# Autobot37/weatherforecastingtoolkit

Measured on AMD Instinct MI355X. Metric: SEVIR 384x384 frames/sec (AE train step), higher is better.
Workload: dtype f32; 1 GPU; experiments/ae_v2 conv AE (ae_64x8x8_lin.PosAwareAE_TF, img_size=384), 1x384x384 synthetic SEVIR frames, batch 32/GPU, fp32, fwd + L1 + bwd + AdamW + cosine-warmup LR; batch_per_gpu=32, global_batch=32, img_size=384, parallelism=dp1, params=215033281

## Files before the change

### include/wfae.h

```cpp
#ifndef WFAE_H
#define WFAE_H

#include <stddef.h>
#include <stdint.h>

#ifdef __cplusplus
extern "C" {
#endif

typedef void* wfae_stream_t;

typedef enum {
  WFAE_OK = 0,
  WFAE_ERR_BAD_SHAPE = -1,
  WFAE_ERR_NULL_POINTER = -2,
  WFAE_ERR_WORKSPACE = -3,
  WFAE_ERR_LAUNCH = -4,
  WFAE_ERR_UNSUPPORTED = -5
} wfae_status;

int wfae_version(void);
const char* wfae_last_error_string(void);
size_t wfae_workspace_bytes(int64_t max_weight_elems);

// ... 4 lines not shown
int wfae_set_split_gemm(int on);
int wfae_get_split_gemm(void);

int wfae_set_c1n(int on);
int wfae_get_c1n(void);

int wfae_conv1x1_fwd(const float* x, const float* w, const float* bias, const float* res,
                     int64_t res_img_stride, float* y, int NB, int Cin, int Cout, int HW,
                     wfae_stream_t stream);
int wfae_conv1x1_fwd_stats(const float* x, const float* w, const float* bias, const float* res,
                           int64_t res_img_stride, float* y, int NB, int Cin, int Cout, int HW,
                           double* stat_part, int64_t stat_capacity, int* stat_rows, wfae_stream_t stream);
int wfae_conv1x1_fwd_bnact(const float* x, const float* bn_scale, const float* bn_shift, const float* w,
                           const float* bias, const float* res, int64_t res_img_stride, float* y, int NB, int Cin,
                           int Cout, int HW, double* stat_part, int64_t stat_capacity, int* stat_rows,
                           wfae_stream_t stream);
int wfae_conv1x1_bwd_weight_bnact(const float* dy, const float* x, const float* bn_scale, const float* bn_shift,
                                  float* dw, int NB, int Cin, int Cout, int HW, int accumulate, void* ws,
                                  size_t ws_bytes, wfae_stream_t stream);
int wfae_conv1x1_bwd_data(const float* dy, const float* w, float* dx, int NB, int Cin, int Cout,
                          int HW, wfae_stream_t stream);
int wfae_conv1x1_bwd_weight(const float* dy, const float* x, float* dw, int NB, int Cin, int Cout,
                            int HW, int accumulate, void* ws, size_t ws_bytes, wfae_stream_t stream);

int wfae_c1r_supported(int M, int K, int HW);
int wfae_c1r_stat_rows(int M, int K, int NB, int HW);
int wfae_c1r_fwd(const float* w, int64_t w_sm, int64_t w_sk, const float* x, const float* pro_scale, const float* pro_shift,
                 const float* res, float* y, int NB, int K, int M, int HW, double* stat_part, int64_t stat_capacity,
                 int* stat_rows, wfae_stream_t stream);
int wfae_c1r_bnred_supported(int M, int K, int HW);
int wfae_c1r_bnred(const float* w, int64_t w_sm, int64_t w_sk, const float* dt, const float* x, const float* bn_scale,
                   const float* bn_shift, const float* save_mean, const float* save_invstd, float* da, int NB, int K, int M, int HW,
                   double* part, int64_t part_capacity, int* part_rows, wfae_stream_t stream);
int wfae_bn_act_bwd_from_rows(const double* part, int rows, int C, float* dgamma, float* dbeta, int accumulate, void* ws,
                              size_t ws_bytes, wfae_stream_t stream);
int wfae_c1r_bndx(const float* w, int64_t w_sm, int64_t w_sk, const float* dt, const float* x, const float* gamma,
                  const float* bn_scale, const float* bn_shift, const float* save_mean, const float* save_invstd, const float* coef,
                  const float* res, float* dx, int NB, int K, int M, int HW, int training, wfae_stream_t stream);
int wfae_c1rb_supported(int M, int K, int HW);
int wfae_c1rb_stat_rows(int M, int K, int NB, int HW);
int wfae_c1rb_fwd(const float* w, int64_t w_sm, int64_t w_sk, const uint16_t* x, const float* pro_scale, const float* pro_shift,
                  const uint16_t* res, uint16_t* y, int NB, int K, int M, int HW, double* stat_part, int64_t stat_capacity,
                  int* stat_rows, wfae_stream_t stream);
int wfae_c1w_supported(int Cin, int Cout, int HW);
int wfae_c1w_bwd_weight(const float* dy, const float* x, const float* bn_scale, const float* bn_shift, float* dw, int NB, int Cin,
                        int Cout, int HW, int accumulate, void* ws, size_t ws_bytes, wfae_stream_t stream);
int wfae_c1w_bwd_weight_bf16(const uint16_t* dy, const uint16_t* x, const float* bn_scale, const float* bn_shift, float* dw, int NB,
                             int Cin, int Cout, int HW, int accumulate, void* ws, size_t ws_bytes, wfae_stream_t stream);
int wfae_set_c1wd(int on);
int wfae_get_c1wd(void);
int wfae_c1wd_supported(int C, int mid, int HW);
int wfae_c1wd_bwd(const float* dy, const float* t2, const float* bn_scale, const float* bn_shift, const float* w3, float* dw3,
                  float* da3, int NB, int C, int mid, int HW, int accumulate, void* ws, size_t ws_bytes, wfae_stream_t stream);
int wfae_set_c1ws(int on);
int wfae_get_c1ws(void);
int wfae_c1ws_supported(int C, int mid, int HW);
int wfae_c1ws_stat_rows(int C, int mid, int NB, int HW, size_t ws_bytes);
int wfae_c1ws_bwd(const float* x, const float* dt1, const float* bn_scale, const float* bn_shift, const float* save_mean,
                  const float* save_invstd, const float* w1, float* dw1, double* part, int64_t part_capacity, int* part_rows, int NB,
                  int C, int mid, int HW, int accumulate, void* ws, size_t ws_bytes, wfae_stream_t stream);
int wfae_linear_fwd(const float* x, const float* w, const float* bias, float* y, int B, int In,
                    int Out, void* ws, size_t ws_bytes, wfae_stream_t stream);
int wfae_linear_bwd_data(const float* dy, const float* w, float* dx, int B, int In, int Out,
                         wfae_stream_t stream);
int wfae_linear_bwd_weight(const float* dy, const float* x, float* dw, int B, int In, int Out,
                           int accumulate, wfae_stream_t stream);
int wfae_linear_bwd_data_splitk(const float* dy, const float* w, float* dx, int B, int In, int Out, void* ws,
                                size_t ws_bytes, wfae_stream_t stream);
int wfae_linear_bwd_weight_splitk(const float* dy, const float* x, float* dw, int B, int In, int Out, int accumulate,
                                  void* ws, size_t ws_bytes, wfae_stream_t stream);

int wfae_conv4x4s2_down(const float* hi, const float* w, float* lo, int NB, int Chi, int Clo,
                        int Hlo, int Wlo, wfae_stream_t stream);
int wfae_conv4x4s2_up(const float* lo, const float* w, float* hi, int NB, int Chi, int Clo, int Hlo,
                      int Wlo, void* ws, size_t ws_bytes, wfae_stream_t stream);
int wfae_conv4x4s2_wgrad(const float* lo, const float* hi, float* dw, int NB, int Chi, int Clo,
                         int Hlo, int Wlo, int accumulate, void* ws, size_t ws_bytes,
                         wfae_stream_t stream);

int wfae_dconv_fwd(const float* x, const float* w, const float* bias, float* y, int NB, int Cin,
                   int Cout, int H, int W, int KS, int stride, int pad, int groups,
                   wfae_stream_t stream);
int wfae_dconv_bwd_data(const float* dy, const float* w, float* dx, int NB, int Cin, int Cout,
                        int H, int W, int KS, int pad, int groups, wfae_stream_t stream);
int wfae_dconv_bwd_weight(const float* dy, const float* x, float* dw, int NB, int Cin, int Cout,
                          int H, int W, int KS, int stride, int pad, int groups, int accumulate,
                          void* ws, size_t ws_bytes, wfae_stream_t stream);

int wfae_gconv3x3_fwd(const float* x, const float* w, float* y, int NB, int C, int H, int W, int groups,
                      int transposed, void* ws, size_t ws_bytes, wfae_stream_t stream);
int wfae_gconv3x3_bwd_weight(const float* dy, const float* x, float* dw, int NB, int C, int H, int W,
                             int groups, int accumulate, void* ws, size_t ws_bytes, wfae_stream_t stream);

int wfae_bn_stats_train(const float* x, int NB, int C, int HW, const float* gamma,
                        const float* beta, float eps, float momentum, float* running_mean,
                        float* running_var, float* save_mean, float* save_invstd, float* scale,
                        float* shift, void* ws, size_t ws_bytes, wfae_stream_t stream);
int wfae_bn_stats_from_rows(const double* stat_part, int rows, int NB, int C, int HW, const float* gamma,
                            const float* beta, float eps, float momentum, float* running_mean,
                            float* running_var, float* save_mean, float* save_invstd, float* scale,
                            float* shift, void* ws, size_t ws_bytes, wfae_stream_t stream);
int wfae_bn_fold_eval(const float* gamma, const float* beta, const float* running_mean,
                      const float* running_var, float eps, float* save_mean, float* save_invstd,
                      float* scale, float* shift, int C, wfae_stream_t stream);
int wfae_bn_act_fwd(const float* x, const float* scale, const float* shift, float* y, int NB, int C,
                    int HW, int act, wfae_stream_t stream);
// ... 361 lines not shown
```

### weatherforecastingtoolkit_amd/csrc/c1wd.hip

```cpp
#include "common.h"
#include <atomic>
#include <stdlib.h>
#include <type_traits>

using namespace wfae;

namespace {

typedef float f32x4 __attribute__((ext_vector_type(4)));
typedef float f32x16 __attribute__((ext_vector_type(16)));
typedef __bf16 bf16x8 __attribute__((ext_vector_type(8)));
typedef short s16x4 __attribute__((ext_vector_type(4)));
typedef short s16x8 __attribute__((ext_vector_type(8)));
typedef unsigned u32x4 __attribute__((ext_vector_type(4)));
typedef unsigned u32x2 __attribute__((ext_vector_type(2)));

struct C1WDP {
  const float* dy;
  const float* t2;
  const float* w3;
  const float* pro_scale;
  const float* pro_shift;
  float* slab;
  float* da;
  int HW;
  int cpi;
  int kc;
};

constexpr int DNT = 512, DBK = 32;

__device__ __forceinline__ unsigned off_row(int r, int c) { return (unsigned)(r * 64 + ((c ^ ((r >> 2) & 3)) << 4)); }

__device__ __forceinline__ void split_pair(float a, float b, unsigned& h, unsigned& m, unsigned& l) {
  h = pack_bf16(a, b);
  const float ra = a - bf16_lo(h), rb = b - bf16_hi(h);
  m = pack_bf16(ra, rb);
  l = pack_bf16(ra - bf16_lo(m), rb - bf16_hi(m));
}

template <int C>
__global__ __launch_bounds__(DNT, C == 128 ? 4 : 2) void c1wd_kernel(C1WDP p) {
  constexpr int M = C / 4;
  constexpr int TM = C / 128;
  constexpr int WQ = M / 32;
  constexpr int NDW = 4 * WQ;
  constexpr bool BOTH = NDW == 8;
  constexpr int KCH = C / 32;
  constexpr int LPR = 8;
  constexpr int P_LD = C * LPR, Q_LD = M * LPR;
  constexpr int P_IT = P_LD / DNT;
  static_assert(P_LD % DNT == 0 && Q_LD <= DNT, "loader");
  constexpr int A_PLANE_B = C * 64, B_PLANE_B = M * 64;
  constexpr int A_STAGE_B = 3 * A_PLANE_B, STAGE_B = 3 * (A_PLANE_B + B_PLANE_B);
  __shared__ __attribute__((aligned(16))) unsigned char smem[2 * STAGE_B];
  const int t = threadIdx.x, lane = t & 63;
  const int wave = __builtin_amdgcn_readfirstlane(t >> 6);
  const int img = blockIdx.x / p.cpi, chunk = blockIdx.x - img * p.cpi;
  const int k_begin = chunk * p.kc;
  const int k_end = min(p.HW, k_begin + p.kc);
  const int nsteps = (k_end - k_begin) / DBK;
  const bool do_dw = BOTH || wave < NDW, do_da = BOTH || wave >= NDW;

  const float* Pb = p.dy + (long)img * C * p.HW + k_begin;
  const float* Qb = p.t2 + (long)img * M * p.HW + k_begin;
  const float* p_src[P_IT];
  unsigned p_dst[P_IT];
#pragma unroll
  for (int j = 0; j < P_IT; ++j) {
    const int idx = t + j * DNT, r = idx / LPR, e = idx % LPR;
    p_src[j] = Pb + (long)r * p.HW + e * 4;
    p_dst[j] = off_row(r, e >> 1) + (unsigned)((e & 1) * 8);
  }
  const bool q_on = Q_LD == DNT || t < Q_LD;
  const int q_r = q_on ? t / LPR : 0, q_e = t % LPR;
  const float* q_src = Qb + (long)q_r * p.HW + q_e * 4;
  const unsigned q_dst = off_row(q_r, q_e >> 1) + (unsigned)((q_e & 1) * 8);
  const float q_s = p.pro_scale[q_r], q_h = p.pro_shift[q_r];
  u32x4 rp[P_IT], rq;
  auto load_global = [&]() {
#pragma unroll
    for (int j = 0; j < P_IT; ++j) rp[j] = *reinterpret_cast<const u32x4*>(p_src[j]);
    if (q_on) rq = *reinterpret_cast<const u32x4*>(q_src);
  };
  auto advance = [&](bool more) {
#pragma unroll
    for (int j = 0; j < P_IT; ++j) p_src[j] += more ? DBK : 0;
    q_src += more ? DBK : 0;
  };
  auto put = [&](unsigned char* base, int plane_b, unsigned dst, u32x4 r, bool act, float s, float h) {
    const unsigned u0 = r[0], u1 = r[1], u2 = r[2], u3 = r[3];
    float v0 = __uint_as_float(u0), v1 = __uint_as_float(u1), v2 = __uint_as_float(u2), v3 = __uint_as_float(u3);
    if (act) {
      v0 = gelu_f(fmaf(v0, s, h)); v1 = gelu_f(fmaf(v1, s, h));
      v2 = gelu_f(fmaf(v2, s, h)); v3 = gelu_f(fmaf(v3, s, h));
    }
    unsigned h0, m0, l0, h1, m1, l1;
    split_pair(v0, v1, h0, m0, l0);
    split_pair(v2, v3, h1, m1, l1);
    *reinterpret_cast<u32x2*>(base + dst) = u32x2{h0, h1};
    *reinterpret_cast<u32x2*>(base + plane_b + dst) = u32x2{m0, m1};
    *reinterpret_cast<u32x2*>(base + 2 * plane_b + dst) = u32x2{l0, l1};
  };
  auto store_lds = [&](int buf) {
    unsigned char* s = smem + buf * STAGE_B;
#pragma unroll
    for (int j = 0; j < P_IT; ++j) put(s, A_PLANE_B, p_dst[j], rp[j], false, 0.f, 0.f);
    if (q_on) put(s + A_STAGE_B, B_PLANE_B, q_dst, rq, true, q_s, q_h);
  };

  const int wm0 = (BOTH ? (wave >> 1) : (wave & 3)) * (32 * TM), wn0 = BOTH ? (wave & 1) * 32 : 0;
  const int r31 = lane & 31, lh = lane >> 5;
  const unsigned a_rd = (unsigned)((wm0 + r31) * 64), b_rd = (unsigned)((wn0 + r31) * 64);
  const int a_x = (r31 >> 2) & 3;
  f32x16 acc[TM];
  struct Frag {
    bf16x8 a[TM][3], b[3];
  };
  auto read_frag = [&](Frag& f, int buf, int ks) {
    const unsigned char* s = smem + buf * STAGE_B;
    const unsigned a_c = (unsigned)(((2 * ks + lh) ^ a_x) << 4);
#pragma unroll
    for (int i = 0; i < TM; ++i)
#pragma unroll
      for (int pl = 0; pl < 3; ++pl)
        f.a[i][pl] = *reinterpret_cast<const bf16x8*>(s + pl * A_PLANE_B + a_rd + i * (32 * 64) + a_c);
#pragma unroll
    for (int pl = 0; pl < 3; ++pl) f.b[pl] = *reinterpret_cast<const bf16x8*>(s + A_STAGE_B + pl * B_PLANE_B + b_rd + a_c);
  };
  auto mfma_frag = [&](const Frag& f) {
#pragma unroll
    for (int i = 0; i < TM; ++i) {
      f32x16 c = acc[i];
      c = __builtin_amdgcn_mfma_f32_32x32x16_bf16(f.a[i][2], f.b[0], c, 0, 0, 0);
      c = __builtin_amdgcn_mfma_f32_32x32x16_bf16(f.a[i][0], f.b[2], c, 0, 0, 0);
      c = __builtin_amdgcn_mfma_f32_32x32x16_bf16(f.a[i][1], f.b[1], c, 0, 0, 0);
      c = __builtin_amdgcn_mfma_f32_32x32x16_bf16(f.a[i][1], f.b[0], c, 0, 0, 0);
      c = __builtin_amdgcn_mfma_f32_32x32x16_bf16(f.a[i][0], f.b[1], c, 0, 0, 0);
      c = __builtin_amdgcn_mfma_f32_32x32x16_bf16(f.a[i][0], f.b[0], c, 0, 0, 0);
      acc[i] = c;
    }
  };

  const int dtile = BOTH ? wave : (wave & 3);
  const int mt = dtile >> 1, pt = dtile & 1;
  const int n16 = lane & 15, kg = lane >> 4, tq = n16 >> 2, tp = n16 & 3;
  bf16x8 wa[KCH][3];
  auto load_weights = [&]() {
#pragma unroll
    for (int ch = 0; ch < KCH; ++ch) {
      const float* src = p.w3 + (long)(32 * ch + 8 * kg) * M + 16 * mt + n16;
      float v[8];
#pragma unroll
      for (int e = 0; e < 8; ++e) v[e] = src[e * M];
      u32x4 h, m, l;
#pragma unroll
      for (int e = 0; e < 4; ++e) {
        unsigned qh, qm, ql;
        split_pair(v[2 * e], v[2 * e + 1], qh, qm, ql);
        h[e] = qh; m[e] = qm; l[e] = ql;
      }
      wa[ch][0] = __builtin_bit_cast(bf16x8, h);
      wa[ch][1] = __builtin_bit_cast(bf16x8, m);
      wa[ch][2] = __builtin_bit_cast(bf16x8, l);
    }
  };
  unsigned tr_rd[2];
#pragma unroll
  for (int hf = 0; hf < 2; ++hf) tr_rd[hf] = off_row(8 * kg + 4 * hf + tq, 2 * pt + (tp >> 1)) + 8u * (unsigned)(tp & 1);
  float* const da_dst = p.da + ((long)img * M + 16 * mt + 4 * kg) * p.HW + k_begin + 16 * pt + n16;
  auto da_step = [&](int buf, int st) {
    const unsigned char* s = smem + buf * STAGE_B;
    constexpr int PA[6] = {2, 0, 1, 1, 0, 0}, PB[6] = {0, 2, 1, 0, 1, 0};
    f32x4 d = {0.f, 0.f, 0.f, 0.f};
#pragma unroll
    for (int ch = 0; ch < KCH; ++ch) {
      bf16x8 b[3];
#pragma unroll
      for (int pl = 0; pl < 3; ++pl) {
        s16x4 part[2];
#pragma unroll
        for (int hf = 0; hf < 2; ++hf)
          part[hf] = __builtin_amdgcn_ds_read_tr16_b64_v4i16(
              (s16x4 __attribute__((address_space(3)))*)(s + pl * A_PLANE_B + ch * (32 * 64) + tr_rd[hf]));
        b[pl] = __builtin_bit_cast(bf16x8, __builtin_shufflevector(part[0], part[1], 0, 1, 2, 3, 4, 5, 6, 7));
      }
#pragma unroll
      for (int pr = 0; pr < 6; ++pr) d = __builtin_amdgcn_mfma_f32_16x16x32_bf16(wa[ch][PA[pr]], b[PB[pr]], d, 0, 0, 0);
    }
    float* o = da_dst + 32 * st;
#pragma unroll
    for (int q = 0; q < 4; ++q) o[(long)q * p.HW] = d[q];
  };

  auto run = [&](auto dwc, auto dac) {
    constexpr bool DW = decltype(dwc)::value, DA = decltype(dac)::value;
    if constexpr (DW) {
#pragma unroll
      for (int i = 0; i < TM; ++i)
#pragma unroll
        for (int q = 0; q < 16; ++q) acc[i][q] = 0.f;
    }
    if constexpr (DA) load_weights();
    if (nsteps > 0) {
      Frag f0, f1;
      load_global();
      advance(nsteps > 1);
      store_lds(0);
      load_global();
      advance(nsteps > 2);
      __syncthreads();
      if constexpr (DW) read_frag(f0, 0, 0);
      for (int st = 0; st < nsteps; ++st) {
        const int cur = st & 1;
        if constexpr (DW) read_frag(f1, cur, 1);
        store_lds(cur ^ 1);
        load_global();
        advance(st + 3 < nsteps);
        if constexpr (DW) mfma_frag(f0);
        if constexpr (DA) da_step(cur, st);
        __builtin_amdgcn_sched_barrier(0);
        __syncthreads();
        __builtin_amdgcn_sched_barrier(0);
        if constexpr (DW) {
          read_frag(f0, cur ^ 1, 0);
          mfma_frag(f1);
        }
        __builtin_amdgcn_sched_barrier(0);
      }
    }
    if constexpr (DW) {
      float* __restrict__ Cb = p.slab + (long)blockIdx.x * C * M;
#pragma unroll
      for (int i = 0; i < TM; ++i)
#pragma unroll
        for (int q = 0; q < 16; ++q) {
          const int row = wm0 + 32 * i + (q & 3) + 8 * (q >> 2) + 4 * lh;
          Cb[(long)row * M + wn0 + r31] = acc[i][q];
        }
    }
  };
  if constexpr (BOTH) run(std::true_type{}, std::true_type{});
  else if (do_dw) run(std::true_type{}, std::false_type{});
  else run(std::false_type{}, std::true_type{});
}

std::atomic<int> g_c1wd{-1};
inline bool c1wd_on() {
  int v = g_c1wd.load(std::memory_order_relaxed);
  if (v < 0) {
    const char* e = getenv("WFAE_C1WD");
    v = (e && e[0] == '0') ? 0 : 1;
    g_c1wd.store(v, std::memory_order_relaxed);
  }
  return v == 1;
}

inline bool al16(const void* q) { return (reinterpret_cast<uintptr_t>(q) & 15) == 0; }

inline bool c1wd_shape_ok(int C, int mid, int HW) { return (C == 128 || C == 256) && mid * 4 == C && HW > 0 && HW % 64 == 0; }

}

extern "C" {

int wfae_set_c1wd(int on) {
  g_c1wd.store(on ? 1 : 0, std::memory_order_relaxed);
  return WFAE_OK;
}

int wfae_get_c1wd(void) { return c1wd_on() ? 1 : 0; }

int wfae_c1wd_supported(int C, int mid, int HW) {
  return (c1wd_on() && c1wd_shape_ok(C, mid, HW) && wfae::split_gemm_enabled()) ? 1 : 0;
}

int wfae_c1wd_bwd(const float* dy, const float* t2, const float* bn_scale, const float* bn_shift, const float* w3, float* dw3,
                  float* da3, int NB, int C, int mid, int HW, int accumulate, void* ws, size_t ws_bytes, wfae_stream_t stream) {
  WFAE_REQUIRE(dy && t2 && bn_scale && bn_shift && w3 && dw3 && da3 && ws, WFAE_ERR_NULL_POINTER, "c1wd_bwd: null pointer");
  WFAE_REQUIRE(NB > 0 && C > 0 && mid > 0 && HW > 0 && NB <= 65535 && (int64_t)NB * HW < (1ll << 31), WFAE_ERR_BAD_SHAPE,
               "c1wd_bwd: bad shape");
  WFAE_REQUIRE(c1wd_shape_ok(C, mid, HW), WFAE_ERR_UNSUPPORTED,
               "c1wd_bwd: serves C = 128 or 256 with mid = C / 4 and HW %% 64 == 0 (C %d, mid %d, HW %d)", C, mid, HW);
  WFAE_REQUIRE(c1wd_on() && wfae::split_gemm_enabled(), WFAE_ERR_UNSUPPORTED,
               "c1wd_bwd: needs fp32 precision with the split GEMMs on and wfae_set_c1wd(1)");
  WFAE_REQUIRE(al16(dy) && al16(t2), WFAE_ERR_UNSUPPORTED, "c1wd_bwd: dy and t2 must be 16-byte aligned");
  C1WDP p = {};
  p.dy = dy; p.t2 = t2; p.w3 = w3;
  p.pro_scale = bn_scale; p.pro_shift = bn_shift;
  p.slab = (float*)ws; p.da = da3;
  p.HW = HW;
  WFAE_REQUIRE(c1w_chunks(C, mid, NB, HW, ws_bytes, &p.cpi, &p.kc), WFAE_ERR_WORKSPACE, "c1wd_bwd: workspace %zu < %zu", ws_bytes,
               (size_t)NB * C * mid * sizeof(float));
  hipStream_t st = (hipStream_t)stream;
  const dim3 grid((unsigned)(NB * p.cpi)), block(DNT);
  if (C == 128) hipLaunchKernelGGL((c1wd_kernel<128>), grid, block, 0, st, p);
  else hipLaunchKernelGGL((c1wd_kernel<256>), grid, block, 0, st, p);
  const int rc = check_launch("c1wd_bwd");
  if (rc) return rc;
  return slab_reduce((const float*)ws, dw3, nullptr, (long)C * mid, mid, NB * p.cpi, accumulate, st, 0);
}

}
```

### weatherforecastingtoolkit_amd/functional.py

```python
from __future__ import annotations

import os

import torch
from torch.autograd import Function

from . import ops

BN_EPS = 1e-5


_overlap = False
_side = {}


STAT_FUSION = os.environ.get("WFAE_STAT_FUSION", "1") == "1"


FUSE_A1 = os.environ.get("WFAE_FUSE_A1", "1") == "1"
FUSE_A1_MAXC = 1 << 30
FUSE_A3 = os.environ.get("WFAE_FUSE_A3", "1") == "1"
FUSE_A3_MAXC = int(os.environ.get("WFAE_FUSE_A3_MAXC", "128"))
FUSE_A3_MAXC_C1R = max(FUSE_A3_MAXC, 256)

# ... 471 lines not shown
class BottleneckFn(Function):
    @staticmethod
    def forward(ctx, x, g1, b1, w1, g2, b2, wg, g3, b3, w3, mod, x_stats=None):
        xc = _c(x)
        if xc is not x:
            x_stats = None
        x = xc
        bn1, bn2, bn3 = mod.f[0], mod.f[3], mod.f[6]
        groups = mod.f[5].groups
        training = _use_batch_stats(bn1)
        fuse = training and STAT_FUSION
        emit = fuse and getattr(mod, "emit_stats", False)
        C, mid, hw = x.shape[1], w1.shape[0], x.shape[2] * x.shape[3]
        sto = _storage(x)

        def route(op, m, k, pro=False, res="none"):
            return ops.conv1x1_route(op, m, k, hw, sto, pro, False, res)
        fused1 = FUSE_A1 and C <= FUSE_A1_MAXC and ops.conv1x1_bnact_supported(x, mid)
        r1, r3 = route("fwd", mid, C, fused1), route("fwd", C, mid, True, "ordinary")
        fused3 = (FUSE_A3 and C <= (FUSE_A3_MAXC_C1R if r3 in ("c1r", "c1rb") else FUSE_A3_MAXC)
                  and ops.conv1x1_bnact_supported((x.shape[0], mid) + x.shape[2:], C))
        if not fused3:
            r3 = route("fwd", C, mid, False, "ordinary")
        d1, d3 = (route("dgrad", C, mid), route("dgrad", mid, C)) if sto == "bf16" else (None, None)
        W1p, W3p = (ops.c1b_weights(w1), ops.c1b_weights(w3)) if "c1b" in (r1, r3, d1, d3) else ((None, None), (None, None))
        st1 = _bn_stats_rows(x_stats if (fuse or isinstance(x_stats, ops.StatParts)) else None, x, bn1, training)
        a1 = None if fused1 else ops.bn_act_fwd(x, st1, 1)
        t1, sr2 = _c1(w1, W1p[0], False, *((x, st1) if fused1 else (a1, None)), None, fuse, r1)
        st2 = _bn_stats_rows(sr2, t1, bn2, training)
        a2 = ops.bn_act_fwd(t1, st2, 1)
        t2 = _g3_fwd(a2, wg, groups)
        st3 = _bn_stats(t2, bn3, training)
        a3 = None if fused3 else ops.bn_act_fwd(t2, st3, 1)
        y, mod._out_stats = _c1(w3, W3p[0], False, *((t2, st3) if fused3 else (a3, None)), x, emit, r3)
        ctx.save_for_backward(x, _opt(a1), t1, a2, t2, _opt(a3), g1, w1, g2, wg, g3, w3,
                              st1.mean, st1.invstd, st1.scale, st1.shift,
                              st2.mean, st2.invstd, st2.scale, st2.shift,
                              st3.mean, st3.invstd, st3.scale, st3.shift,
                              _opt(W1p[1] if d1 == "c1b" else None), _opt(W3p[1] if d3 == "c1b" else None))
        ctx.training = training
        ctx.groups = groups
        ctx.betas = (b1, b2, b3)
        return y

    @staticmethod
    def backward(ctx, dy):
        (x, a1, t1, a2, t2, a3, g1, w1, g2, wg, g3, w3, *s) = ctx.saved_tensors
        st1, st2, st3 = _mk_stats(*s[0:4]), _mk_stats(*s[4:8]), _mk_stats(*s[8:12])
        W1t, W3t = s[12], s[13]
        tr = ctx.training
        dy = _c(dy)
        mid = w1.shape[0]
        dw3 = grad_buffer(w3)
        da3 = None
        if a3.numel() == 0:
            if ops.conv1x1_wd_route(dy.shape[1], mid, dy.shape[2] * dy.shape[3], _storage(dy)) == "c1wd":
                da3 = _on_main(lambda: ops.conv1x1_bwd_wd(dy, t2, st3, w3, dw3))
            if da3 is None:
                _wgrad(lambda: ops.conv1x1_bwd_weight_bnact(dy, t2, st3, dw3), dy, t2, st3.scale, st3.shift)
        else:
            _wgrad(lambda: ops.conv1x1_bwd_weight(dy, a3, dw3), dy, a3)
        dg3, db3 = grad_buffer(g3), grad_buffer(ctx.betas[2])
        if da3 is not None:
            dt2 = ops.bn_act_bwd(da3, t2, g3, st3, dg3, db3, None, 1, tr)
        else:
            dt2 = _dgrad_bn(dy, w3, W3t, t2, g3, st3, dg3, db3, None, tr)
        del da3
        dwg = grad_buffer(wg)
        _wgrad(lambda: _g3_wgrad(dt2, a2, dwg, ctx.groups), dt2, a2)
        da2 = _g3_dgrad(dt2, wg, mid, ctx.groups)
        del dt2
        dg2, db2 = grad_buffer(g2), grad_buffer(ctx.betas[1])
        dt1 = ops.bn_act_bwd(da2, t1, g2, st2, dg2, db2, None, 1, tr)
        del da2
        dw1 = grad_buffer(w1)
        rows1 = None
        if a1.numel() == 0:
            if ops.conv1x1_ws_route(x.shape[1], mid, x.shape[2] * x.shape[3], _storage(x)) == "c1ws":
                rows1 = _on_main(lambda: ops.conv1x1_bwd_ws(dt1, x, st1, w1, dw1))
            if rows1 is None:
                _wgrad(lambda: ops.conv1x1_bwd_weight_bnact(dt1, x, st1, dw1), dt1, x, st1.scale, st1.shift)
        else:
            _wgrad(lambda: ops.conv1x1_bwd_weight(dt1, a1, dw1), dt1, a1)
        dg1, db1 = grad_buffer(g1), grad_buffer(ctx.betas[0])
        dx = _dgrad_bn(dt1, w1, W1t, x, g1, st1, dg1, db1, dy, tr, rows1)
        return dx, dg1, db1, dw1, dg2, db2, dwg, dg3, db3, dw3, None, None


class Conv1x1Fn(Function):

    @staticmethod
    def forward(ctx, x, w, bias, pos):
        ctx.x_dtype = x.dtype
        x = ops.to_f32(_c(x))
        y = ops.conv1x1_fwd(x, w, bias, None if pos is None else _c(pos), pos is not None)
        ctx.save_for_backward(x, w)
        ctx.bias, ctx.pos = bias, pos
        return y

    @staticmethod
    def backward(ctx, dy):
        x, w = ctx.saved_tensors
        dy = ops.to_f32(_c(dy))
        nb, cout, h, wd = dy.shape
        dw = grad_buffer(w)
        ops.conv1x1_bwd_weight(dy, x, dw)
        dx = ops.to_dtype(ops.conv1x1_bwd_data(dy, w), ctx.x_dtype) if ctx.needs_input_grad[0] else None
        dbias = dpos = None
        if ctx.bias is not None:
            dbias = grad_buffer(ctx.bias)
            ops.reduce_sum(dy, nb, cout, h * wd, dbias)
        if ctx.pos is not None:
            dpos = grad_buffer(ctx.pos)
            ops.reduce_sum(dy, nb, cout * h * wd, 1, dpos)
        return dx, dw, dbias, dpos

# ... 1034 lines not shown
```

### weatherforecastingtoolkit_amd/ops.py

```python
from __future__ import annotations

import ctypes
import math
import os

import torch

from . import _lib

_WS_DEFAULT = int(os.environ.get("WFAE_WORKSPACE_MB", "512")) << 20
_ws = {}


def _stream():
    return torch.cuda.current_stream().cuda_stream


_prof = None


def profile_start():
    global _prof
    _prof = {}

# ... 159 lines not shown
def _p(t):
    return None if t is None else t.data_ptr()


class StatRows:
    __slots__ = ("part", "rows")

    def __init__(self, part, rows):
        self.part, self.rows = part, rows


class StatParts:
    __slots__ = ("part", "splits")

    def __init__(self, part, splits):
        self.part, self.splits = part, splits


def _rows_out(n, device):
    part = torch.empty(n, dtype=torch.float64, device=device)
    count = ctypes.c_int(0)
    return part, count, (part.data_ptr(), n, ctypes.cast(ctypes.pointer(count), ctypes.c_void_p))


_NO_ROWS = (None, 0, None)


_C1R = _C1R_BNRED = _C1R_BNDX = _C1RB = _C1B = _C1W = True


def set_c1r(on):
    global _C1R
    _C1R = bool(on)


def set_c1r_bnred(on):
    global _C1R_BNRED
    _C1R_BNRED = bool(on)


def set_c1r_bndx(on):
    global _C1R_BNDX
    _C1R_BNDX = bool(on)


def set_c1n(on):
    _lib.call("wfae_set_c1n", int(bool(on)))


def set_c1wd(on):
    _lib.call("wfae_set_c1wd", int(bool(on)))


def set_c1ws(on):
    _lib.call("wfae_set_c1ws", int(bool(on)))


def set_c1rb(on):
    global _C1RB
    _C1RB = bool(on)


def set_c1b(on):
    global _C1B
    _C1B = bool(on)


def set_c1w(on):
    global _C1W
    _C1W = bool(on)


def c1r_bndx_on():
    return _C1R_BNDX


def c1n_enabled():
    return bool(_lib.load().wfae_get_c1n())


def c1wd_enabled():
    return bool(_lib.load().wfae_get_c1wd())


def c1ws_enabled():
    return bool(_lib.load().wfae_get_c1ws())


def _precision():
    return _lib.load().wfae_get_matmul_precision()


def c1r_supported(m, k, hw):
    return _C1R and _SPLIT_GEMM and _precision() == 0 and bool(_lib.load().wfae_c1r_supported(int(m), int(k), int(hw)))


def c1r_bnred_supported(m, k, hw):
    return (_C1R and _C1R_BNRED and _SPLIT_GEMM and _precision() == 0
            and bool(_lib.load().wfae_c1r_bnred_supported(int(m), int(k), int(hw))))


def c1rb_supported(m, k, hw):
    return _C1RB and _precision() == 1 and bool(_lib.load().wfae_c1rb_supported(int(m), int(k), int(hw)))


def c1b_supported(m, k, hw):
    return _C1B and _precision() == 1 and bool(_lib.load().wfae_c1b_supported(int(m), int(k), int(hw)))


def conv1x1_bnact_supported(x, cout):
    nb, cin, h, wd = getattr(x, "shape", x)
    swapped = cin < cout and cin < 128
    return (h * wd) % 4 == 0 and h * wd >= 16 and cin % 4 == 0 and (cout % 4 == 0 or not swapped)


def conv1x1_route(op, m, k, hw, storage="f32", prologue=False, bias=False, residual="none"):
    if op == "wgrad":
        ok = _C1W and _lib.load().wfae_c1w_supported(int(k), int(m), int(hw))
        return "c1w" if ok and (_precision() == 1 if storage == "bf16" else (_precision() == 0 and _SPLIT_GEMM)) else "gemm"
    if bias or residual == "broadcast" or (residual == "ordinary" and m <= k):
        return "gemm"
    if storage == "f32":
        return "c1r" if c1r_supported(m, k, hw) else "gemm"
    rb = c1rb_supported(m, k, hw)
    if rb and not (prologue and m < k and k >= 256):
        return "c1rb"
    return "c1b" if (rb or c1b_supported(m, k, hw)) else "gemm"


def conv1x1_dgrad_bn_route(m, k, hw, storage="f32"):
    if storage == "f32" and c1r_bnred_supported(m, k, hw):
        return "bndx" if _C1R_BNDX else "bnred"
    return None


# ... 112 lines not shown
        name, peak = "wfae_c1w_bwd_weight" + sfx, PEAK_BF16_MFMA / (1 if sfx else 6)
    elif sfx:
        name = "wfae_conv1x1_bwd_weight_bf16"
    else:
        name, pro = ("wfae_conv1x1_bwd_weight", ()) if st is None else ("wfae_conv1x1_bwd_weight_bnact", pro)
    ws = workspace()
    _call(name, 2 * n * cin * cout, es * n * (cin + cout) + 4 * cin * cout, _p(dy), _p(x), *pro, _p(dw), nb, cin, cout, h * wd,
          int(accumulate), ws.data_ptr(), ws.numel(), _stream(), peak=peak,
          label="wfae_conv1x1_bwd_weight" if st is None else "wfae_conv1x1_bwd_weight_bnact")
    return dw


def conv1x1_bwd_weight(dy, x, dw, accumulate=False):
    return _c1_wgrad(dy, x, None, dw, accumulate)


def conv1x1_bwd_weight_bnact(dy, x, st, dw, accumulate=False):
    return _c1_wgrad(dy, x, st, dw, accumulate)


C1WD_MIN_HW = 512


def conv1x1_wd_supported(c, mid, hw, storage="f32"):
    return (storage == "f32" and _SPLIT_GEMM and _precision() == 0 and bool(_lib.load().wfae_c1wd_supported(int(c), int(mid), int(hw)))
            and conv1x1_route("wgrad", c, mid, hw, "f32", True) == "c1w" and conv1x1_route("dgrad", mid, c, hw) == "c1r")


def conv1x1_wd_route(c, mid, hw, storage="f32"):
    return "c1wd" if hw >= C1WD_MIN_HW and conv1x1_wd_supported(c, mid, hw, storage) else "pair"


def conv1x1_bwd_wd(dy, t2, st, w3, dw3, accumulate=False):
    if st is None or dy.dtype != torch.float32 or t2.dtype != torch.float32:
        return None
    nb, c, h, wd = dy.shape
    mid, hw = t2.shape[1], h * wd
    if not conv1x1_wd_supported(c, mid, hw):
        return None
    _chk(dy, t2, w3, dw3)
    if tuple(t2.shape) != (nb, mid, h, wd) or w3.numel() != c * mid or dw3.numel() != c * mid:
        raise _lib.WfaeError("conv1x1_bwd_wd: dy (N, C, H, W), t2 (N, C/4, H, W), w3 and dw3 (C, C/4)")
    if (dy.data_ptr() | t2.data_ptr()) & 15:
        return None
    da = torch.empty_like(t2)
    n = nb * hw
    ws = workspace()
    _call("wfae_c1wd_bwd", 4 * n * c * mid, 4 * n * (c + 2 * mid) + 8 * c * mid, _p(dy), _p(t2), _p(st.scale), _p(st.shift), _p(w3),
          _p(dw3), _p(da), nb, c, mid, hw, int(accumulate), ws.data_ptr(), ws.numel(), _stream(), peak=PEAK_BF16_MFMA / 6,
          label="wfae_c1wd_bwd")
    return da


def conv1x1_ws_supported(c, mid, hw, storage="f32"):
    return (storage == "f32" and _SPLIT_GEMM and _precision() == 0 and bool(_lib.load().wfae_c1ws_supported(int(c), int(mid), int(hw)))
            and conv1x1_route("wgrad", mid, c, hw, "f32", True) == "c1w" and conv1x1_dgrad_bn_route(c, mid, hw, storage) == "bndx")


def conv1x1_ws_route(c, mid, hw, storage="f32"):
    return "c1ws" if hw >= C1WD_MIN_HW and conv1x1_ws_supported(c, mid, hw, storage) else "pair"


def conv1x1_bwd_ws(dt1, x, st, w1, dw1, accumulate=False):
    if st is None or dt1.dtype != torch.float32 or x.dtype != torch.float32:
        return None
    nb, c, h, wd = x.shape
    mid, hw = dt1.shape[1], h * wd
    if not conv1x1_ws_supported(c, mid, hw):
        return None
    _chk(dt1, x, w1, dw1)
    if tuple(dt1.shape) != (nb, mid, h, wd) or w1.numel() != c * mid or dw1.numel() != c * mid:
        raise _lib.WfaeError("conv1x1_bwd_ws: x (N, C, H, W), dt1 (N, C/4, H, W), w1 and dw1 (C/4, C)")
    if (dt1.data_ptr() | x.data_ptr()) & 15:
        return None
    n = nb * hw
    ws = workspace()
    cap = 2 * int(_lib.load().wfae_c1ws_stat_rows(c, mid, nb, hw, ws.numel())) * c
    if cap <= 0:
        return None
    part, rows, out = _rows_out(cap, x.device)
    _call("wfae_c1ws_bwd", 4 * n * c * mid, 4 * n * (c + mid) + 8 * c * mid, _p(x), _p(dt1), _p(st.scale), _p(st.shift), _p(st.mean),
          _p(st.invstd), _p(w1), _p(dw1), *out, nb, c, mid, hw, int(accumulate), ws.data_ptr(), ws.numel(), _stream(),
          peak=PEAK_BF16_MFMA / 6, label="wfae_c1ws_bwd")
    return StatRows(part[:2 * rows.value * c], rows.value)


def c1r_bnred(w, dt, x, st, store=True):
    _chk(w, dt, x)
    nb, k, h, wd = dt.shape
    m, n = w.shape[1], nb * h * wd
    da = torch.empty((nb, m, h, wd), dtype=torch.float32, device=dt.device) if store else None
    part, rows, out = _rows_out(2 * int(_lib.load().wfae_c1r_stat_rows(m, k, nb, h * wd)) * m, dt.device)
    _call("wfae_c1r_bnred", 2 * n * k * m, 4 * (n * (k + (2 if store else 1) * m) + k * m), _p(w), 1, m, _p(dt), _p(x), _p(st.scale),
          _p(st.shift), _p(st.mean), _p(st.invstd), _p(da), nb, k, m, h * wd, *out, _stream(), label="wfae_conv1x1_bwd_data",
          peak=_C1_PEAK["c1r"])
    return da, StatRows(part[:2 * rows.value * m], rows.value)


def bn_act_bwd_from_rows(sr, c, dgamma, dbeta, accumulate=False):
    _chk(dgamma, dbeta)
    ws = workspace()
    _call("wfae_bn_act_bwd_from_rows", 0, 8 * sr.part.numel(), sr.part.data_ptr(), sr.rows, c, _p(dgamma), _p(dbeta), int(accumulate),
          ws.data_ptr(), ws.numel(), _stream(), label="wfae_bn_act_bwd[reduce]")
    return ws


# ... 2004 lines not shown
```

Baseline: 182.9 frames/s.

## Fuse batchnorm-backward reductions into the c1wd weight/data-grad kernel

```diff
diff --git a/include/wfae.h b/include/wfae.h
--- a/include/wfae.h
+++ b/include/wfae.h
@@ -80,6 +80,14 @@
 int wfae_c1wd_supported(int C, int mid, int HW);
 int wfae_c1wd_bwd(const float* dy, const float* t2, const float* bn_scale, const float* bn_shift, const float* w3, float* dw3,
                   float* da3, int NB, int C, int mid, int HW, int accumulate, void* ws, size_t ws_bytes, wfae_stream_t stream);
+int wfae_set_c1wd_sums(int on);
+int wfae_get_c1wd_sums(void);
+int wfae_c1wd_sums_supported(int C, int mid, int HW);
+int wfae_c1wd_sums_stat_rows(int C, int mid, int NB, int HW, size_t ws_bytes);
+int wfae_c1wd_bwd_sums(const float* dy, const float* t2, const float* bn_scale, const float* bn_shift, const float* save_mean,
+                       const float* save_invstd, const float* w3, float* dw3, float* da3, double* part, int64_t part_capacity,
+                       int* part_rows, int NB, int C, int mid, int HW, int accumulate, void* ws, size_t ws_bytes,
+                       wfae_stream_t stream);
 int wfae_set_c1ws(int on);
 int wfae_get_c1ws(void);
 int wfae_c1ws_supported(int C, int mid, int HW);
diff --git a/weatherforecastingtoolkit_amd/csrc/c1wd.hip b/weatherforecastingtoolkit_amd/csrc/c1wd.hip
--- a/weatherforecastingtoolkit_amd/csrc/c1wd.hip
+++ b/weatherforecastingtoolkit_amd/csrc/c1wd.hip
@@ -21,14 +21,19 @@
   const float* w3;
   const float* pro_scale;
   const float* pro_shift;
+  const float* mean;
+  const float* invstd;
   float* slab;
   float* da;
+  double* part0;
+  double* part1;
   int HW;
   int cpi;
   int kc;
 };
 
 constexpr int DNT = 512, DBK = 32;
+constexpr int D_LD = 20;
 
 __device__ __forceinline__ unsigned off_row(int r, int c) { return (unsigned)(r * 64 + ((c ^ ((r >> 2) & 3)) << 4)); }
 
@@ -39,7 +44,7 @@
   l = pack_bf16(ra - bf16_lo(m), rb - bf16_hi(m));
 }
 
-template <int C>
+template <int C, bool SUMS>
 __global__ __launch_bounds__(DNT, C == 128 ? 4 : 2) void c1wd_kernel(C1WDP p) {
   constexpr int M = C / 4;
   constexpr int TM = C / 128;
@@ -53,7 +58,9 @@
   static_assert(P_LD % DNT == 0 && Q_LD <= DNT, "loader");
   constexpr int A_PLANE_B = C * 64, B_PLANE_B = M * 64;
   constexpr int A_STAGE_B = 3 * A_PLANE_B, STAGE_B = 3 * (A_PLANE_B + B_PLANE_B);
-  __shared__ __attribute__((aligned(16))) unsigned char smem[2 * STAGE_B];
+  constexpr int D_WAVE_B = 16 * D_LD * 4;
+  constexpr int D_ALL_B = SUMS ? (BOTH ? 8 : 4) * D_WAVE_B : 0;
+  __shared__ __attribute__((aligned(16))) unsigned char smem[2 * STAGE_B + D_ALL_B];
   const int t = threadIdx.x, lane = t & 63;
   const int wave = __builtin_amdgcn_readfirstlane(t >> 6);
   const int img = blockIdx.x / p.cpi, chunk = blockIdx.x - img * p.cpi;
@@ -61,6 +68,8 @@
   const int k_end = min(p.HW, k_begin + p.kc);
   const int nsteps = (k_end - k_begin) / DBK;
   const bool do_dw = BOTH || wave < NDW, do_da = BOTH || wave >= NDW;
+  const int dtile = BOTH ? wave : (wave & 3);
+  const int mt = dtile >> 1, pt = dtile & 1;
 
   const float* Pb = p.dy + (long)img * C * p.HW + k_begin;
   const float* Qb = p.t2 + (long)img * M * p.HW + k_begin;
@@ -72,15 +81,21 @@
     p_src[j] = Pb + (long)r * p.HW + e * 4;
     p_dst[j] = off_row(r, e >> 1) + (unsigned)((e & 1) * 8);
   }
-  const bool q_on = Q_LD == DNT || t < Q_LD;
-  const int q_r = q_on ? t / LPR : 0, q_e = t % LPR;
+  const bool q_on = SUMS ? do_da : (Q_LD == DNT || t < Q_LD);
+  const int q_r = SUMS ? 16 * mt + (lane >> 2) : (q_on ? t / LPR : 0), q_e = SUMS ? 4 * pt + (lane & 3) : t % LPR;
   const float* q_src = Qb + (long)q_r * p.HW + q_e * 4;
   const unsigned q_dst = off_row(q_r, q_e >> 1) + (unsigned)((q_e & 1) * 8);
   const float q_s = p.pro_scale[q_r], q_h = p.pro_shift[q_r];
+  float q_mu = 0.f, q_is = 0.f;
+  if constexpr (SUMS) { q_mu = p.mean[q_r]; q_is = p.invstd[q_r]; }
   u32x4 rp[P_IT], rq;
-  auto load_global = [&]() {
+  float gp[4], xh[4];
+  double sum1 = 0.0, sum2 = 0.0;
+  auto load_p = [&]() {
 #pragma unroll
     for (int j = 0; j < P_IT; ++j) rp[j] = *reinterpret_cast<const u32x4*>(p_src[j]);
+  };
+  auto load_q = [&]() {
     if (q_on) rq = *reinterpret_cast<const u32x4*>(q_src);
   };
   auto advance = [&](bool more) {
@@ -102,11 +117,28 @@
     *reinterpret_cast<u32x2*>(base + plane_b + dst) = u32x2{m0, m1};
     *reinterpret_cast<u32x2*>(base + 2 * plane_b + dst) = u32x2{l0, l1};
   };
-  auto store_lds = [&](int buf) {
+  auto store_p = [&](int buf) {
     unsigned char* s = smem + buf * STAGE_B;
 #pragma unroll
     for (int j = 0; j < P_IT; ++j) put(s, A_PLANE_B, p_dst[j], rp[j], false, 0.f, 0.f);
-    if (q_on) put(s + A_STAGE_B, B_PLANE_B, q_dst, rq, true, q_s, q_h);
+  };
+  auto store_q = [&](int buf) {
+    unsigned char* s = smem + buf * STAGE_B + A_STAGE_B;
+    if constexpr (!SUMS) {
+      if (q_on) put(s, B_PLANE_B, q_dst, rq, true, q_s, q_h);
+    } else if (q_on) {
+      const unsigned u0 = rq[0], u1 = rq[1], u2 = rq[2], u3 = rq[3];
+      const float x0 = __uint_as_float(u0), x1 = __uint_as_float(u1), x2 = __uint_as_float(u2), x3 = __uint_as_float(u3);
+      const float w0 = fmaf(x0, q_s, q_h), w1 = fmaf(x1, q_s, q_h), w2 = fmaf(x2, q_s, q_h), w3 = fmaf(x3, q_s, q_h);
+      gp[0] = gelu_grad_f(w0); gp[1] = gelu_grad_f(w1); gp[2] = gelu_grad_f(w2); gp[3] = gelu_grad_f(w3);
+      xh[0] = (x0 - q_mu) * q_is; xh[1] = (x1 - q_mu) * q_is; xh[2] = (x2 - q_mu) * q_is; xh[3] = (x3 - q_mu) * q_is;
+      unsigned h0, m0, l0, h1, m1, l1;
+      split_pair(gelu_f(w0), gelu_f(w1), h0, m0, l0);
+      split_pair(gelu_f(w2), gelu_f(w3), h1, m1, l1);
+      *reinterpret_cast<u32x2*>(s + q_dst) = u32x2{h0, h1};
+      *reinterpret_cast<u32x2*>(s + B_PLANE_B + q_dst) = u32x2{m0, m1};
+      *reinterpret_cast<u32x2*>(s + 2 * B_PLANE_B + q_dst) = u32x2{l0, l1};
+    }
   };
 
   const int wm0 = (BOTH ? (wave >> 1) : (wave & 3)) * (32 * TM), wn0 = BOTH ? (wave & 1) * 32 : 0;
@@ -142,8 +174,6 @@
     }
   };
 
-  const int dtile = BOTH ? wave : (wave & 3);
-  const int mt = dtile >> 1, pt = dtile & 1;
   const int n16 = lane & 15, kg = lane >> 4, tq = n16 >> 2, tp = n16 & 3;
   bf16x8 wa[KCH][3];
   auto load_weights = [&]() {
@@ -168,6 +198,9 @@
   unsigned tr_rd[2];
 #pragma unroll
   for (int hf = 0; hf < 2; ++hf) tr_rd[hf] = off_row(8 * kg + 4 * hf + tq, 2 * pt + (tp >> 1)) + 8u * (unsigned)(tp & 1);
+  unsigned char* const dwave = smem + 2 * STAGE_B + (SUMS ? dtile * D_WAVE_B : 0);
+  float* const d_wr = reinterpret_cast<float*>(dwave) + (4 * kg) * D_LD + n16;
+  const unsigned char* const d_rd = dwave + ((lane >> 2) * D_LD + 4 * (lane & 3)) * 4;
   float* const da_dst = p.da + ((long)img * M + 16 * mt + 4 * kg) * p.HW + k_begin + 16 * pt + n16;
   auto da_step = [&](int buf, int st) {
     const unsigned char* s = smem + buf * STAGE_B;
@@ -191,6 +224,25 @@
     float* o = da_dst + 32 * st;
 #pragma unroll
     for (int q = 0; q < 4; ++q) o[(long)q * p.HW] = d[q];
+    if constexpr (SUMS) {
+#pragma unroll
+      for (int q = 0; q < 4; ++q) d_wr[q * D_LD] = d[q];
+    }
+  };
+  auto sums_step = [&]() {
+    __builtin_amdgcn_fence(__ATOMIC_RELEASE, "wavefront");
+    __builtin_amdgcn_wave_barrier();
+    __builtin_amdgcn_fence(__ATOMIC_ACQUIRE, "wavefront");
+    const f32x4 v = *reinterpret_cast<const f32x4*>(d_rd);
+    const float d0 = v.x * gp[0], d1 = v.y * gp[1];
+    const float d2 = v.z * gp[2], d3 = v.w * gp[3];
+    const float h0 = xh[0], h1 = xh[1], h2 = xh[2], h3 = xh[3];
+    const float s1 = (d0 + d1) + (d2 + d3);
+    const float s2 = fmaf(d0, h0, d1 * h1) + fmaf(d2, h2, d3 * h3);
+    sum1 += (double)s1;
+    sum2 += (double)s2;
+    __builtin_amdgcn_fence(__ATOMIC_RELEASE, "wavefront");
+    __builtin_amdgcn_wave_barrier();
   };
 
   auto run = [&](auto dwc, auto dac) {
@@ -202,6 +254,15 @@
         for (int q = 0; q < 16; ++q) acc[i][q] = 0.f;
     }
     if constexpr (DA) load_weights();
+    constexpr bool QW = !SUMS || DA;
+    auto load_global = [&]() {
+      load_p();
+      if constexpr (QW) load_q();
+    };
+    auto store_lds = [&](int buf) {
+      store_p(buf);
+      if constexpr (QW) store_q(buf);
+    };
     if (nsteps > 0) {
       Frag f0, f1;
       load_global();
@@ -210,19 +271,36 @@
       load_global();
       advance(nsteps > 2);
       __syncthreads();
-      if constexpr (DW) read_frag(f0, 0, 0);
+      constexpr bool LATE = SUMS && DW && DA;
+      if constexpr (DW && !LATE) read_frag(f0, 0, 0);
       for (int st = 0; st < nsteps; ++st) {
         const int cur = st & 1;
+        if constexpr (LATE) read_frag(f0, cur, 0);
         if constexpr (DW) read_frag(f1, cur, 1);
-        store_lds(cur ^ 1);
-        load_global();
-        advance(st + 3 < nsteps);
-        if constexpr (DW) mfma_frag(f0);
-        if constexpr (DA) da_step(cur, st);
+        if constexpr (SUMS && DA) {
+          store_p(cur ^ 1);
+          load_p();
+          if constexpr (LATE) {
+            mfma_frag(f0);
+            mfma_frag(f1);
+            __builtin_amdgcn_sched_barrier(0);
+          }
+          da_step(cur, st);
+          sums_step();
+          store_q(cur ^ 1);
+          load_q();
+          advance(st + 3 < nsteps);
+        } else {
+          store_lds(cur ^ 1);
+          load_global();
+          advance(st + 3 < nsteps);
+          if constexpr (DW) mfma_frag(f0);
+          if constexpr (DA) da_step(cur, st);
+        }
         __builtin_amdgcn_sched_barrier(0);
         __syncthreads();
         __builtin_amdgcn_sched_barrier(0);
-        if constexpr (DW) {
+        if constexpr (DW && !LATE) {
           read_frag(f0, cur ^ 1, 0);
           mfma_frag(f1);
         }
@@ -243,6 +321,29 @@
   if constexpr (BOTH) run(std::true_type{}, std::true_type{});
   else if (do_dw) run(std::true_type{}, std::false_type{});
   else run(std::false_type{}, std::true_type{});
+
+  if constexpr (SUMS) {
+    double e1 = sum1, e2 = sum2;
+#pragma unroll
+    for (int o = 1; o < 4; o <<= 1) {
+      e1 += __shfl_xor(e1, o, 64);
+      e2 += __shfl_xor(e2, o, 64);
+    }
+    double* const tot = reinterpret_cast<double*>(dwave);
+    const int r = lane >> 2;
+    const bool owner = do_da && (lane & 3) == 0;
+    if (owner) {
+      tot[2 * r] = e1;
+      tot[2 * r + 1] = e2;
+    }
+    __syncthreads();
+    if (owner && pt == 0) {
+      const double* const hi = reinterpret_cast<const double*>(dwave + D_WAVE_B);
+      const long at = (long)blockIdx.x * M + 16 * mt + r;
+      p.part0[at] = tot[2 * r] + hi[2 * r];
+      p.part1[at] = tot[2 * r + 1] + hi[2 * r + 1];
+    }
+  }
 }
 
 std::atomic<int> g_c1wd{-1};
@@ -258,7 +359,59 @@
 
 inline bool al16(const void* q) { return (reinterpret_cast<uintptr_t>(q) & 15) == 0; }
 
+std::atomic<int> g_c1wd_sums{-1};
+inline bool c1wd_sums_on() {
+  int v = g_c1wd_sums.load(std::memory_order_relaxed);
+  if (v < 0) {
+    const char* e = getenv("WFAE_C1WD_SUMS");
+    v = (e && e[0] == '0') ? 0 : 1;
+    g_c1wd_sums.store(v, std::memory_order_relaxed);
+  }
+  return v == 1;
+}
+
 inline bool c1wd_shape_ok(int C, int mid, int HW) { return (C == 128 || C == 256) && mid * 4 == C && HW > 0 && HW % 64 == 0; }
+
+int c1wd_launch(const char* what, const float* dy, const float* t2, const float* bn_scale, const float* bn_shift, const float* mean,
+                const float* invstd, const float* w3, float* dw3, float* da3, double* part, int64_t part_capacity, int* part_rows,
+                int NB, int C, int mid, int HW, int accumulate, void* ws, size_t ws_bytes, wfae_stream_t stream) {
+  WFAE_REQUIRE(dy && t2 && bn_scale && bn_shift && w3 && dw3 && da3 && ws, WFAE_ERR_NULL_POINTER, "%s: null pointer", what);
+  WFAE_REQUIRE(NB > 0 && C > 0 && mid > 0 && HW > 0 && NB <= 65535 && (int64_t)NB * HW < (1ll << 31), WFAE_ERR_BAD_SHAPE,
+               "%s: bad shape", what);
+  WFAE_REQUIRE(c1wd_shape_ok(C, mid, HW), WFAE_ERR_UNSUPPORTED,
+               "%s: serves C = 128 or 256 with mid = C / 4 and HW %% 64 == 0 (C %d, mid %d, HW %d)", what, C, mid, HW);
+  WFAE_REQUIRE(c1wd_on() && wfae::split_gemm_enabled(), WFAE_ERR_UNSUPPORTED,
+               "%s: needs fp32 precision with the split GEMMs on and wfae_set_c1wd(1)", what);
+  WFAE_REQUIRE(al16(dy) && al16(t2), WFAE_ERR_UNSUPPORTED, "%s: dy and t2 must be 16-byte aligned", what);
+  C1WDP p = {};
+  p.dy = dy; p.t2 = t2; p.w3 = w3;
+  p.pro_scale = bn_scale; p.pro_shift = bn_shift;
+  p.mean = mean; p.invstd = invstd;
+  p.slab = (float*)ws; p.da = da3;
+  p.HW = HW;
+  WFAE_REQUIRE(c1w_chunks(C, mid, NB, HW, ws_bytes, &p.cpi, &p.kc), WFAE_ERR_WORKSPACE, "%s: workspace %zu < %zu", what, ws_bytes,
+               (size_t)NB * C * mid * sizeof(float));
+  const int rows = NB * p.cpi;
+  if (part) {
+    WFAE_REQUIRE(part_capacity >= 2 * (int64_t)rows * mid, WFAE_ERR_WORKSPACE, "%s: part holds %lld doubles, needs %lld", what,
+                 (long long)part_capacity, (long long)(2 * (int64_t)rows * mid));
+    *part_rows = rows;
+    p.part0 = part;
+    p.part1 = part + (long)rows * mid;
+  }
+  hipStream_t st = (hipStream_t)stream;
+  const dim3 grid((unsigned)rows), block(DNT);
+  if (part) {
+    if (C == 128) hipLaunchKernelGGL((c1wd_kernel<128, true>), grid, block, 0, st, p);
+    else hipLaunchKernelGGL((c1wd_kernel<256, true>), grid, block, 0, st, p);
+  } else {
+    if (C == 128) hipLaunchKernelGGL((c1wd_kernel<128, false>), grid, block, 0, st, p);
+    else hipLaunchKernelGGL((c1wd_kernel<256, false>), grid, block, 0, st, p);
+  }
+  const int rc = check_launch(what);
+  if (rc) return rc;
+  return slab_reduce((const float*)ws, dw3, nullptr, (long)C * mid, mid, rows, accumulate, st, 0);
+}
 
 }
 
@@ -277,28 +430,33 @@
 
 int wfae_c1wd_bwd(const float* dy, const float* t2, const float* bn_scale, const float* bn_shift, const float* w3, float* dw3,
                   float* da3, int NB, int C, int mid, int HW, int accumulate, void* ws, size_t ws_bytes, wfae_stream_t stream) {
-  WFAE_REQUIRE(dy && t2 && bn_scale && bn_shift && w3 && dw3 && da3 && ws, WFAE_ERR_NULL_POINTER, "c1wd_bwd: null pointer");
-  WFAE_REQUIRE(NB > 0 && C > 0 && mid > 0 && HW > 0 && NB <= 65535 && (int64_t)NB * HW < (1ll << 31), WFAE_ERR_BAD_SHAPE,
-               "c1wd_bwd: bad shape");
-  WFAE_REQUIRE(c1wd_shape_ok(C, mid, HW), WFAE_ERR_UNSUPPORTED,
-               "c1wd_bwd: serves C = 128 or 256 with mid = C / 4 and HW %% 64 == 0 (C %d, mid %d, HW %d)", C, mid, HW);
-  WFAE_REQUIRE(c1wd_on() && wfae::split_gemm_enabled(), WFAE_ERR_UNSUPPORTED,
-               "c1wd_bwd: needs fp32 precision with the split GEMMs on and wfae_set_c1wd(1)");
-  WFAE_REQUIRE(al16(dy) && al16(t2), WFAE_ERR_UNSUPPORTED, "c1wd_bwd: dy and t2 must be 16-byte aligned");
-  C1WDP p = {};
-  p.dy = dy; p.t2 = t2; p.w3 = w3;
-  p.pro_scale = bn_scale; p.pro_shift = bn_shift;
-  p.slab = (float*)ws; p.da = da3;
-  p.HW = HW;
-  WFAE_REQUIRE(c1w_chunks(C, mid, NB, HW, ws_bytes, &p.cpi, &p.kc), WFAE_ERR_WORKSPACE, "c1wd_bwd: workspace %zu < %zu", ws_bytes,
-               (size_t)NB * C * mid * sizeof(float));
-  hipStream_t st = (hipStream_t)stream;
-  const dim3 grid((unsigned)(NB * p.cpi)), block(DNT);
-  if (C == 128) hipLaunchKernelGGL((c1wd_kernel<128>), grid, block, 0, st, p);
-  else hipLaunchKernelGGL((c1wd_kernel<256>), grid, block, 0, st, p);
-  const int rc = check_launch("c1wd_bwd");
-  if (rc) return rc;
-  return slab_reduce((const float*)ws, dw3, nullptr, (long)C * mid, mid, NB * p.cpi, accumulate, st, 0);
-}
-
-}
+  return c1wd_launch("c1wd_bwd", dy, t2, bn_scale, bn_shift, nullptr, nullptr, w3, dw3, da3, nullptr, 0, nullptr, NB, C, mid, HW,
+                     accumulate, ws, ws_bytes, stream);
+}
+
+int wfae_set_c1wd_sums(int on) {
+  g_c1wd_sums.store(on ? 1 : 0, std::memory_order_relaxed);
+  return WFAE_OK;
+}
+
+int wfae_get_c1wd_sums(void) { return c1wd_sums_on() ? 1 : 0; }
+
+int wfae_c1wd_sums_supported(int C, int mid, int HW) { return (c1wd_sums_on() && wfae_c1wd_supported(C, mid, HW)) ? 1 : 0; }
+
+int wfae_c1wd_sums_stat_rows(int C, int mid, int NB, int HW, size_t ws_bytes) {
+  int cpi = 0, kc = 0;
+  if (!c1wd_shape_ok(C, mid, HW) || NB <= 0 || !c1w_chunks(C, mid, NB, HW, ws_bytes, &cpi, &kc)) return 0;
+  return NB * cpi;
+}
+
+int wfae_c1wd_bwd_sums(const float* dy, const float* t2, const float* bn_scale, const float* bn_shift, const float* save_mean,
+                       const float* save_invstd, const float* w3, float* dw3, float* da3, double* part, int64_t part_capacity,
+                       int* part_rows, int NB, int C, int mid, int HW, int accumulate, void* ws, size_t ws_bytes,
+                       wfae_stream_t stream) {
+  WFAE_REQUIRE(save_mean && save_invstd && part && part_rows, WFAE_ERR_NULL_POINTER, "c1wd_bwd_sums: null pointer");
+  WFAE_REQUIRE(c1wd_sums_on(), WFAE_ERR_UNSUPPORTED, "c1wd_bwd_sums: needs wfae_set_c1wd_sums(1)");
+  return c1wd_launch("c1wd_bwd_sums", dy, t2, bn_scale, bn_shift, save_mean, save_invstd, w3, dw3, da3, part, part_capacity,
+                     part_rows, NB, C, mid, HW, accumulate, ws, ws_bytes, stream);
+}
+
+}
diff --git a/weatherforecastingtoolkit_amd/functional.py b/weatherforecastingtoolkit_amd/functional.py
--- a/weatherforecastingtoolkit_amd/functional.py
+++ b/weatherforecastingtoolkit_amd/functional.py
@@ -547,16 +547,26 @@
         dy = _c(dy)
         mid = w1.shape[0]
         dw3 = grad_buffer(w3)
-        da3 = None
+        da3 = rows3 = None
         if a3.numel() == 0:
-            if ops.conv1x1_wd_route(dy.shape[1], mid, dy.shape[2] * dy.shape[3], _storage(dy)) == "c1wd":
+            how3 = ops.conv1x1_wds_route(dy.shape[1], mid, dy.shape[2] * dy.shape[3], _storage(dy))
+            if how3 == "c1wds":
+                got = _on_main(lambda: ops.conv1x1_bwd_wds(dy, t2, st3, w3, dw3))
+                if got is not None:
+                    da3, rows3 = got
+                else:
+                    how3 = "c1wd"
+            if how3 == "c1wd" and da3 is None:
                 da3 = _on_main(lambda: ops.conv1x1_bwd_wd(dy, t2, st3, w3, dw3))
             if da3 is None:
                 _wgrad(lambda: ops.conv1x1_bwd_weight_bnact(dy, t2, st3, dw3), dy, t2, st3.scale, st3.shift)
         else:
             _wgrad(lambda: ops.conv1x1_bwd_weight(dy, a3, dw3), dy, a3)
         dg3, db3 = grad_buffer(g3), grad_buffer(ctx.betas[2])
-        if da3 is not None:
+        if rows3 is not None:
+            ops.bn_act_bwd_from_rows(rows3, mid, dg3, db3)
+            dt2 = ops.bn_act_bwd_dx(da3, t2, g3, st3, None, 1, tr)
+        elif da3 is not None:
             dt2 = ops.bn_act_bwd(da3, t2, g3, st3, dg3, db3, None, 1, tr)
         else:
             dt2 = _dgrad_bn(dy, w3, W3t, t2, g3, st3, dg3, db3, None, tr)
diff --git a/weatherforecastingtoolkit_amd/ops.py b/weatherforecastingtoolkit_amd/ops.py
--- a/weatherforecastingtoolkit_amd/ops.py
+++ b/weatherforecastingtoolkit_amd/ops.py
@@ -235,6 +235,10 @@
     _lib.call("wfae_set_c1wd", int(bool(on)))
 
 
+def set_c1wd_sums(on):
+    _lib.call("wfae_set_c1wd_sums", int(bool(on)))
+
+
 def set_c1ws(on):
     _lib.call("wfae_set_c1ws", int(bool(on)))
 
@@ -264,6 +268,10 @@
 
 def c1wd_enabled():
     return bool(_lib.load().wfae_get_c1wd())
+
+
+def c1wd_sums_enabled():
+    return bool(_lib.load().wfae_get_c1wd_sums())
 
 
 def c1ws_enabled():
@@ -482,6 +490,41 @@
     return da
 
 
+C1WDS_MIN_HW = 36864
+
+
+def conv1x1_wds_route(c, mid, hw, storage="f32"):
+    how = conv1x1_wd_route(c, mid, hw, storage)
+    if how == "c1wd" and hw >= C1WDS_MIN_HW and bool(_lib.load().wfae_c1wd_sums_supported(int(c), int(mid), int(hw))):
+        return "c1wds"
+    return how
+
+
+def conv1x1_bwd_wds(dy, t2, st, w3, dw3, accumulate=False):
+    if st is None or dy.dtype != torch.float32 or t2.dtype != torch.float32:
+        return None
+    nb, c, h, wd = dy.shape
+    mid, hw = t2.shape[1], h * wd
+    if not (conv1x1_wd_supported(c, mid, hw) and bool(_lib.load().wfae_c1wd_sums_supported(int(c), int(mid), int(hw)))):
+        return None
+    _chk(dy, t2, w3, dw3)
+    if tuple(t2.shape) != (nb, mid, h, wd) or w3.numel() != c * mid or dw3.numel() != c * mid:
+        raise _lib.WfaeError("conv1x1_bwd_wds: dy (N, C, H, W), t2 (N, C/4, H, W), w3 and dw3 (C, C/4)")
+    if (dy.data_ptr() | t2.data_ptr()) & 15:
+        return None
+    n = nb * hw
+    ws = workspace()
+    cap = 2 * int(_lib.load().wfae_c1wd_sums_stat_rows(c, mid, nb, hw, ws.numel())) * mid
+    if cap <= 0:
+        return None
+    da = torch.empty_like(t2)
+    part, rows, out = _rows_out(cap, dy.device)
+    _call("wfae_c1wd_bwd_sums", 4 * n * c * mid, 4 * n * (c + 2 * mid) + 8 * c * mid, _p(dy), _p(t2), _p(st.scale), _p(st.shift),
+          _p(st.mean), _p(st.invstd), _p(w3), _p(dw3), _p(da), *out, nb, c, mid, hw, int(accumulate), ws.data_ptr(), ws.numel(),
+          _stream(), peak=PEAK_BF16_MFMA / 6, label="wfae_c1wd_bwd")
+    return da, StatRows(part[:2 * rows.value * mid], rows.value)
+
+
 def conv1x1_ws_supported(c, mid, hw, storage="f32"):
     return (storage == "f32" and _SPLIT_GEMM and _precision() == 0 and bool(_lib.load().wfae_c1ws_supported(int(c), int(mid), int(hw)))
             and conv1x1_route("wgrad", mid, c, hw, "f32", True) == "c1w" and conv1x1_dgrad_bn_route(c, mid, hw, storage) == "bndx")
```

Result: no change. 183.9 frames/s (median of 6 runs) (+0.5%).
